# B3zaleel/draco-sharp

Hardware: NVIDIA B200
Metric: decoded points/sec (higher is better)
Workload: dtype i32->f32

## Files before the change

### draco_sharp_b200/csrc/dcb_api.cu

```cuda
#include <cuda_runtime.h>
#include <stdint.h>
#include <stdio.h>
#include <chrono>
#include <thread>
#include <mutex>
#include <memory>
#include <string>
#include <stdlib.h>
#include <string.h>

#include <algorithm>
#include <atomic>
#include <map>
#include <new>
#include <tuple>
#include <vector>

#include "dcb_internal.h"
#include "dcb_kernels.h"
#include "dcb_mesh_host.h"
#include "dcb_walk.h"

namespace {

constexpr uint64_t kFrontPad = 256;
constexpr uint64_t kBackPad = 64;
constexpr uint32_t kNumSMsDefault = 148;
constexpr uint32_t kSmemPerSM = 227 * 1024;
constexpr uint32_t kSmemPerCtaReserve = 1024;
constexpr uint64_t kTabArenaBudget = 1ull << 30;
constexpr uint64_t kDefaultPointsPerByte = 4096;

inline uint64_t align_up(uint64_t v, uint64_t a) { return (v + a - 1) / a * a; }

struct EnvFlags {
  bool no_par_post, no_fanout, debug_plan, debug_timing, lutb_full, rans_pc, no_direct, no_fast_tagged, no_threads;
  int ctas_per_sm, pairs, par_run, rec_ka;
  bool no_rec, split;
  EnvFlags() {
    no_par_post = getenv("DCB_NO_PAR_POST") != nullptr;
    no_fanout = getenv("DCB_NO_FANOUT") != nullptr;
    debug_plan = getenv("DCB_DEBUG_PLAN") != nullptr;
    debug_timing = getenv("DCB_DEBUG_TIMING") != nullptr;
    lutb_full = getenv("DCB_LUTB_FULL") != nullptr;
    rans_pc = getenv("DCB_RANS_PC") != nullptr;
    no_direct = getenv("DCB_NO_DIRECT") != nullptr;
    no_threads = getenv("DCB_NO_THREADS") != nullptr;
    no_fast_tagged = getenv("DCB_NO_FAST_TAGGED") != nullptr;
    ctas_per_sm = getenv("DCB_CTAS_PER_SM") ? atoi(getenv("DCB_CTAS_PER_SM")) : 0;
    pairs = getenv("DCB_PAIRS") ? atoi(getenv("DCB_PAIRS")) : 0;
    par_run = getenv("DCB_PAR_RUN") ? atoi(getenv("DCB_PAR_RUN")) : 0;
    no_rec = getenv("DCB_REC") == nullptr;
    split = getenv("DCB_SPLIT") != nullptr;
    rec_ka = getenv("DCB_REC_KA") ? atoi(getenv("DCB_REC_KA")) : 0;
  }
};
const EnvFlags &env_flags() {
  static const EnvFlags f;
  return f;
}

struct PoolBlock {
  void *p;
  uint64_t bytes;
  int device;
};
struct DevPool {
  std::mutex mu;
  std::vector<PoolBlock> free_blocks;
// ... 72 lines not shown
  int share = 1;
  bool arena_pending = false;
  bool maps_pending = false;
  std::shared_ptr<DevPool> pool;
  uint64_t cap_in = 0, cap_out = 0, cap_aux = 0, cap_maps = 0, cap_stage = 0, cap_streams = 0, cap_walks = 0, cap_order = 0;
  int device = 0;
  std::vector<int> bufs;
  std::vector<StreamDesc> streams, streams0;
  std::vector<BufWalk> walks, walks0;
  std::vector<uint8_t> tags_launched;
  PointStage pstage{};
  uint64_t in_bytes = 0, out_bytes = 0, dbg_bytes = 0, aux_bytes = 0, maps_bytes = 0;
  uint64_t out_base = 0, dbg_base = 0;
  uint8_t *d_in = nullptr, *d_out = nullptr, *d_dbg = nullptr, *d_aux = nullptr, *d_tab = nullptr, *d_maps = nullptr;
  uint64_t tab_cap = 0, dbg_cap = 0;
  StreamDesc *d_streams = nullptr;
  BufWalk *d_walks = nullptr;
  uint32_t *d_order = nullptr;
  uint64_t order_cap = 0;
  uint8_t *h_stage = nullptr;
  uint8_t *h_maps = nullptr;
  uint64_t cap_hmaps = 0;
  uint8_t *h_desc = nullptr;
  uint64_t cap_hdesc = 0;
  bool desc_pending = false;
  std::vector<uint32_t> order_host;
  uint32_t epoch = 0;
  bool uploaded = false, dirty = true, own_out = false;
  uint8_t *ext_out = nullptr, *ext_dbg = nullptr;
  std::vector<uint64_t> fin_off, fin_bytes;
// ... 378 lines not shown
}

void pinned_free(const std::shared_ptr<DevPool> &pool, void *p, uint64_t cap);
void free_shard_device(Shard &sh) {
  if (sh.h_desc) {
    pinned_free(sh.pool, sh.h_desc, sh.cap_hdesc);
    sh.h_desc = nullptr;
    sh.desc_pending = false;
  }
  if (!sh.d_in && !sh.d_streams && !sh.h_stage && !sh.d_out && !sh.h_maps) return;
  cudaSetDevice(sh.device);
  pool_free(sh.pool, sh.device, sh.d_in, sh.cap_in);
  if (sh.own_out) pool_free(sh.pool, sh.device, sh.d_out, sh.cap_out);
  cudaFree(sh.d_dbg);
  pool_free(sh.pool, sh.device, sh.d_aux, sh.cap_aux);
  cudaFree(sh.d_tab);
  pool_free(sh.pool, sh.device, sh.d_maps, sh.cap_maps);
  pool_free(sh.pool, sh.device, sh.d_streams, sh.cap_streams);
  pool_free(sh.pool, sh.device, sh.d_walks, sh.cap_walks);
  pool_free(sh.pool, sh.device, sh.d_order, sh.cap_order);
  pool_free(sh.pool, sh.device, sh.d_pts, sh.cap_pts);
  sh.d_pts = nullptr;
  pool_free(sh.pool, sh.device, sh.d_faces, sh.cap_faces);
  sh.d_faces = nullptr;
  if (sh.h_fstatus) pinned_free(sh.pool, sh.h_fstatus, sh.cap_hfstatus);
  sh.h_fstatus = nullptr;
  if (sh.h_stage) pinned_free(sh.pool, sh.h_stage, sh.cap_stage);
  if (sh.h_maps) pinned_free(sh.pool, sh.h_maps, sh.cap_hmaps);
  sh.h_maps = nullptr;
  sh.d_in = sh.d_out = sh.d_dbg = sh.d_aux = sh.d_tab = sh.d_maps = nullptr;
// ... 498 lines not shown
      const uint32_t blk = std::max(16u, ((1u << g.prec_bits) >> 7) << 2);
      const uint64_t cta_raw = (sm_bytes + 1024 / share) / ctas_per_sm;
      const uint64_t cta_fixed = (uint64_t)kSmemPerCtaReserve + g.lut_bytes + blk + 256;
      const uint64_t cta_budget = cta_raw > cta_fixed ? cta_raw - cta_fixed : 0;
      const uint64_t used = (uint64_t)g.lanes * (lane_bytes + blk);
      if (cta_budget > used) {
        const uint64_t spare = (cta_budget - used) / g.lanes;
        g.lutb_bytes = (uint32_t)std::min<uint64_t>((1u << g.prec_bits) >> 1, spare / 16 * 16);
      }
      if (g.lutb_bytes) {
        const uint32_t need = lutb_need();
        if (need != 0xFFFFFFFFu && !env_flags().lutb_full) g.lutb_bytes = std::min<uint32_t>(g.lutb_bytes, need);
      }
    }
  }
}

int ensure_order(Shard &sh, uint64_t n) {
  if (n <= sh.order_cap) return DCB_OK;
  pool_free(sh.pool, sh.device, sh.d_order, sh.cap_order);
  sh.d_order = nullptr;
  sh.order_cap = 0;
  uint8_t *p = nullptr;
  CUDA_TRY(pool_alloc(sh.pool, sh.device, std::max<uint64_t>(n, 1024) * 4, &p, &sh.cap_order));
  sh.d_order = reinterpret_cast<uint32_t *>(p);
  sh.order_cap = std::max<uint64_t>(n, 1024);
  return DCB_OK;
}

void tl_mark(dcb_ctx *ctx, const std::string &name, cudaStream_t s, bool begin);
// ... 687 lines not shown
    if (key.compact) g.exc = std::max(g.exc, s.n_active - std::min(s.n_active, s.dense_prefix));
    g.total_symbols += s.n_entries;
    g.max_entries = std::max(g.max_entries, s.n_entries);
    g.note_table(s);
    g.order.push_back(si);
  }
  std::vector<Group *> rgs;
  for (auto &kv : raw) rgs.push_back(&kv.second);
  bool side_followers = false;
  for (Group *g : rgs) side_followers = side_followers || (g->mode == 3 && rgs.size() > 1);
  for (Group *g : rgs) {
    g->no_direct = g->force_single_warp;
    for (Group *o : rgs)
      if (o != g && o->order.size() >= (size_t)num_sms * 8) g->no_direct = true;
    std::vector<Group *> one{g};
    plan_rans_groups(one, num_sms, (uint32_t)sh.share, side_followers ? 6u * 1024u : 0u);
  }
  uint64_t n_order = 0;
  auto add = [&](Group &g) {
    g.order_off = n_order;
    n_order += g.order.size();
  };
  for (Group *g : rgs) {
    std::stable_sort(g->order.begin(), g->order.end(),
                     [&](uint32_t x, uint32_t y) { return sh.streams[x].n_entries > sh.streams[y].n_entries; });
    add(*g);
  }
  for (int n = 1; n <= 4; ++n) { add(post[n]); add(para[n]); add(cmp[n]); add(par[n]); }
  add(copy);
  add(octs);
  add(octc);
// ... 81 lines not shown
    for (int n = 1; n <= 4; ++n) all.insert(all.end(), par_runs[n].begin(), par_runs[n].end());

    CUDA_TRY(cudaMemcpyAsync(sh.d_order, all.data(), all.size() * 4, cudaMemcpyHostToDevice, st));
  }
  Group *dom = nullptr;
  for (Group *g : rgs)
    if (!dom || g->total_symbols > dom->total_symbols) dom = g;
  const bool fan_out = rgs.size() > 1 && !env_flags().no_fanout;
  bool flag_kernels = !geo.order.empty();
  for (int n = 1; n <= 4; ++n) flag_kernels = flag_kernels || !cmp[n].order.empty();
  const bool flags_early = flag_kernels && !deferred_descs && !env_flags().no_fanout;
  if (fan_out || flags_early) {
    CUDA_TRY(cudaEventRecord(ctx->fork_ev[dev_index], st));
    for (cudaStream_t ss : ctx->side[dev_index]) CUDA_TRY(cudaStreamWaitEvent(ss, ctx->fork_ev[dev_index], 0));
  }
  bool side_used[3] = {false, false, false};
  size_t gi = 0;
  const cudaStream_t st_main = st;
  for (Group *g : rgs) {
    const uint32_t n = (uint32_t)g->order.size();
    const bool is_dom = timed && dev_index == 0 && g == dom;
    cudaStream_t st = st_main;
    if (fan_out && !g->table_global && (g != dom || g->mode == 3)) {
      const size_t k = g->mode == 3 ? 0 : 1 + gi++ % 2;
      st = ctx->side[dev_index][k];
      side_used[k] = true;
    }
    if (env_flags().debug_plan)
      fprintf(stderr, "[dcb plan] raw group ncp=%d wide=%d compact=%u prec=%u entries=%u mode=%u zig=%u: %u streams, %llu symbols, "
                      "k=%u lut=%uB lutb=%uB ent=%uB lanes=%u pairs=%u split=%u direct=%u global=%d rec_ka=%u rec=%uB (need x8: %u %u %u %u, exc %u)\n",
              g->ncp, (int)g->wide, g->compact, g->prec_bits, g->entries, g->mode, g->zig, n,
              (unsigned long long)g->total_symbols, g->lut_shift, g->lut_bytes, g->lutb_bytes, g->ent_bytes, g->lanes, g->pairs, g->split,
              g->direct, (int)g->table_global, g->rec_ka, g->rec_bytes, g->rec_max[0], g->rec_max[1], g->rec_max[2], g->rec_max[3], g->exc_all);
    if (is_dom) CUDA_TRY(cudaEventRecord(ctx->ev[2], st));
    if (g->table_global) {
      const uint64_t slot_bytes = (uint64_t)g->lut_bytes + g->ent_bytes;
      uint64_t per = std::max<uint64_t>(32, std::min<uint64_t>(kTabArenaBudget / slot_bytes, 0xF0000000ull / slot_bytes) / 32 * 32);
      const uint64_t chunk = std::min<uint64_t>(per, align_up(n, 32));
      if (sh.tab_cap < chunk * slot_bytes) {
        cudaFree(sh.d_tab);
        sh.d_tab = nullptr;
        sh.tab_cap = 0;
        CUDA_TRY(cudaMalloc(&sh.d_tab, chunk * slot_bytes));
        sh.tab_cap = chunk * slot_bytes;
      }
      A.tab = sh.d_tab;
      for (uint64_t o = 0; o < n; o += chunk) {
        RansLaunch L{sh.d_streams, sh.d_order + g->order_off + o, (uint32_t)std::min<uint64_t>(chunk, n - o), 32,
                     g->lut_bytes, 0, g->ent_bytes, g->entries, g->exc, g->lut_shift, g->prec_bits, dump, g->compact, g->zig, 0};
        CUDA_TRY(dcb_launch_rans_raw(L, g->ncp, g->wide, true, A, st));
        stats.n_launches++;
      }
    } else {
      RansLaunch L{sh.d_streams, sh.d_order + g->order_off, n, g->lanes, g->lut_bytes, g->lutb_bytes, g->ent_bytes,
                   g->entries, g->exc, g->lut_shift, g->prec_bits, dump, g->compact, g->zig, g->mode};
      tl_begin(g->mode == 1 ? "rans mode1" : g->mode == 2 ? "rans mode2" : g->mode == 3 ? "rans mode3" : g->mode == 4 ? "rans mode4" : "rans mode0", st);
      L.pairs = g->pairs;
      L.direct = g->direct;
      L.rec_ka = g->rec_ka;
      L.rec_bytes = g->rec_bytes;
      L.split = g->split;
      if (g->rec_ka) L.cap_exc = g->exc_all;
      CUDA_TRY(g->rec_ka ? dcb_launch_rans_raw_rec(L, g->ncp, A, st)
               : g->pairs ? dcb_launch_rans_raw_pc(L, g->ncp, A, st) : dcb_launch_rans_raw(L, g->ncp, g->wide, false, A, st));
      tl_end(st);
      stats.n_launches++;
    }
    if (g->mode == 3) {
      tl_begin("oct_chain", st);
      CUDA_TRY(dcb_launch_oct_chain(sh.d_streams, sh.d_order + g->order_off, n, dump, A, st));
      tl_end(st);
      tl_begin("oct_unit", st);
      CUDA_TRY(dcb_launch_oct_unit(sh.d_streams, sh.d_order + g->order_off, n, g->max_entries, A, st));
      tl_end(st);
      stats.n_launches += 2;
    }
    if (is_dom) {
      CUDA_TRY(cudaEventRecord(ctx->ev[3], st));
      ctx->ev_raw = true;
      for (uint32_t si : g->order) {
        const StreamDesc &sd = sh.streams[si];
// ... 6 lines not shown
      Ls.rec_bytes = g->rec_bytes;
      const uint32_t cta_smem = (g->rec_ka ? dcb_rans_rec_smem_bytes(Ls, 4u * (uint32_t)g->ncp)
                                 : g->pairs ? dcb_rans_pc_smem_bytes(Ls, 4u * (uint32_t)g->ncp) : dcb_rans_smem_bytes(Ls, g->table_global)) + kSmemPerCtaReserve;
      const uint64_t per_wave = (uint64_t)num_sms * std::max<uint32_t>(1u, std::min<uint32_t>(32u, (kSmemPerSM + 1024u) / cta_smem)) * g->lanes * std::max(1u, g->pairs);
      stats.n_waves = g->table_global ? 1 : (int32_t)((n + per_wave - 1) / per_wave);
      if (g->rec_ka)
        snprintf(ctx->raw_name, sizeof ctx->raw_name, "rans_raw_rec<ncp=%d,u16,smem,mode=%u,bucket records 2^%u|16|1,%ux%u lanes,%uB>", g->ncp,
                 g->mode, g->rec_ka, g->pairs, g->lanes, g->rec_bytes);
      else if (g->pairs)
        snprintf(ctx->raw_name, sizeof ctx->raw_name, "rans_raw_pc<ncp=%d,u16,smem,mode=%u,%s,%s,%ux%u lanes>", g->ncp, g->mode,
                 g->direct ? "direct slot LUT" : "two-level LUT", g->compact ? "compact" : "dense", g->pairs, g->lanes);
      else
        snprintf(ctx->raw_name, sizeof ctx->raw_name, "rans_raw_fused<ncp=%d,%s,%s,mode=%u,k=%u,%s>", g->ncp,
                 g->wide ? "u32" : "u16", g->table_global ? "global" : "smem", g->mode, g->lut_shift,
                 g->compact ? "compact" : "dense");
    }
    stats.n_streams += (int32_t)n;
  }
  auto launch_flag_kernels = [&](cudaStream_t fs, cudaStream_t gs) -> int {
    for (int n = 1; n <= 4; ++n)
      if (!cmp[n].order.empty()) {
        CUDA_TRY(dcb_launch_cmp_flags(sh.d_streams, sh.d_order + cmp[n].order_off, (uint32_t)cmp[n].order.size(), A, fs));
        stats.n_launches++;
      }
    if (!geo.order.empty()) {
      CUDA_TRY(dcb_launch_geo_flips(sh.d_streams, sh.d_order + geo.order_off, (uint32_t)geo.order.size(), A, gs));
      stats.n_launches++;
    }
    return DCB_OK;
  };
// ... 7 lines not shown
    if (rcm) return rcm;
  }
  auto launch_cmp_deps = [&](cudaStream_t ds) -> int {
    for (int n = 1; n <= 4; ++n)
      if (!cmp[n].order.empty()) {
        CUDA_TRY(dcb_launch_cmp_deps(sh.d_streams, sh.d_order + cmp[n].order_off, (uint32_t)cmp[n].order.size(), cmp[n].max_entries, A, ds));
        stats.n_launches++;
      }
    return DCB_OK;
  };
  if (flags_early) {
    CUDA_TRY(cudaStreamWaitEvent(ctx->side[dev_index][2], ctx->maps_ev[dev_index], 0));
    int rcd = launch_cmp_deps(ctx->side[dev_index][2]);
    if (rcd) return rcd;
  }
  for (int k = 0; k < 3; ++k)
    if (side_used[k]) {
      CUDA_TRY(cudaEventRecord(ctx->join_ev[dev_index][k], ctx->side[dev_index][k]));
      CUDA_TRY(cudaStreamWaitEvent(st, ctx->join_ev[dev_index][k], 0));
    }
  if (!wide.order.empty()) {
    CUDA_TRY(dcb_launch_wide_post(sh.d_streams, sh.d_order + wide.order_off, (uint32_t)wide.order.size(), dump, A, st));
    stats.n_launches++;
  }
  for (int n = 1; n <= 4; ++n) {
    if (!post[n].order.empty()) {
      CUDA_TRY(dcb_launch_serial_post(sh.d_streams, sh.d_order + post[n].order_off, (uint32_t)post[n].order.size(), n, dump, 0, A, st));
      stats.n_launches++;
    }
    if (!par[n].order.empty()) {
      const uint32_t np = (uint32_t)par[n].order.size();
// ... 384 lines not shown
    for (int dev : c->devices) {
      cudaDeviceProp p;
      if (dev < 0 || dev >= count || cudaGetDeviceProperties(&p, dev) != cudaSuccess || p.major != 10) {
        cudaGetLastError();
        dcb_destroy(c);
        return DCB_ERR_NO_DEVICE;
      }
      cudaStream_t st = nullptr;
      if (cudaSetDevice(dev) != cudaSuccess || cudaStreamCreateWithFlags(&st, cudaStreamNonBlocking) != cudaSuccess) {
        cudaGetLastError();
        dcb_destroy(c);
        return DCB_ERR_CUDA;
      }
      c->streams.push_back(st);
      c->own_stream.push_back(true);
      std::vector<cudaStream_t> side(3, nullptr);
      std::vector<cudaEvent_t> jev(3, nullptr);
      cudaEvent_t fev = nullptr;
      int prio_lo = 0, prio_hi = 0;
      cudaDeviceGetStreamPriorityRange(&prio_lo, &prio_hi);
      for (int k = 0; k < 3; ++k) {
        if (k == 0) cudaStreamCreateWithPriority(&side[k], cudaStreamNonBlocking, prio_hi);
        else cudaStreamCreateWithFlags(&side[k], cudaStreamNonBlocking);
        cudaEventCreateWithFlags(&jev[k], cudaEventDisableTiming);
      }
      cudaEventCreateWithFlags(&fev, cudaEventDisableTiming);
      c->side.push_back(side);
      c->join_ev.push_back(jev);
      c->fork_ev.push_back(fev);
      {
        cudaStream_t ci = nullptr, co = nullptr;
        bool own = true;
        for (size_t e = 0; e + 1 < c->streams.size(); ++e)
          if (c->devices[e] == dev) { ci = c->copy_in[e]; co = c->copy_out[e]; own = false; break; }
        if (own) {
          cudaStreamCreateWithFlags(&ci, cudaStreamNonBlocking);
// ... 493 lines not shown
```

### draco_sharp_b200/csrc/dcb_internal.h

```cpp
#pragma once
#include <stdint.h>

#include "../../include/dracob200.h"

#if defined(__CUDACC__)
#define DCB_HD __host__ __device__ __forceinline__
#else
#define DCB_HD inline
#endif

#define DCB_VARINT_CHUNK 4096u

enum : int32_t {
  DT_INT8 = 1, DT_UINT8 = 2, DT_INT16 = 3, DT_UINT16 = 4, DT_INT32 = 5, DT_UINT32 = 6,
  DT_INT64 = 7, DT_UINT64 = 8, DT_FLOAT32 = 9, DT_FLOAT64 = 10, DT_BOOL = 11, DT_COUNT = 12
};
enum : int32_t { SEQ_GENERIC = 0, SEQ_INTEGER = 1, SEQ_QUANTIZATION = 2, SEQ_NORMALS = 3 };
enum : int32_t {
  PRED_NONE = -2, PRED_DIFFERENCE = 0, PRED_PARALLELOGRAM = 1, PRED_CONSTRAINED_MULTI = 4, PRED_TEX_COORDS_PORTABLE = 5,
  PRED_GEOMETRIC_NORMAL = 6, PRED_COUNT = 7
};
enum : int32_t { XF_NONE = -1, XF_DELTA = 0, XF_WRAP = 1, XF_OCT = 2, XF_OCT_CANON = 3, XF_COUNT = 4 };
enum : uint8_t {
  SCHEME_TAGGED = 0,
// ... 164 lines not shown
  uint32_t lutb_bytes;
  uint32_t ent_bytes;
  uint32_t cap_entries;
  uint32_t cap_exc;
  uint32_t lut_shift;
  uint32_t prec_bits;
  uint32_t dump;
  uint32_t compact;
  uint32_t zig;
  uint32_t mode;
  uint32_t pairs;
  uint32_t direct;
  uint32_t rec_ka;
  uint32_t rec_bytes;
  uint32_t split;
};
```

### draco_sharp_b200/csrc/dcb_kernels.cu

```cuda
#include <cuda_runtime.h>
#include <stdint.h>
#include <algorithm>
#include <stdio.h>
#include <stdlib.h>

#include "dcb_device.cuh"
#include "dcb_internal.h"
#include "dcb_kernels.h"
#include "dcb_walk.h"

using namespace dcb;

namespace {

template <int NCP, typename T, bool DUMP, bool TG, int MODE, int TAB, bool SPLIT>
__device__ __forceinline__ void run_tail(RansLane<T, TG> &rl, const TableGeom &geom, const PostParams &pp, uint8_t *optr,
                                         int32_t *dptr, uint32_t dump, uint32_t n_entries, uint32_t g, int32_t *prev);

template <int NCP, typename T, bool DUMP, bool TG, int MODE, int TAB, bool SPLIT>
__device__ __forceinline__ void run_stream(RansLane<T, TG> &rl, const TableGeom &geom, const PostParams &pp, uint8_t *optr,
                                           int32_t *dptr, uint32_t dump, uint32_t n_entries, uint32_t g_min) {
  const int store = store_of<MODE>(pp), dsize = dsize_of<MODE>(pp);
  int32_t prev[NCP];
#pragma unroll
// ... 74 lines not shown
    while (g + 1 < g_min && rl.bytes_left() >= 2u * kGroupBytes + 4u) {
      lean_sp_group<NCP, MODE, false, 1, true>(rl, pp, optr, g, prev, ca_prev, gate, zero);
      ++g;
      rl.template top_up<(kGroupBytes + 15) / 16 + 1>();
      cp_async_wait<1>();
    }
    lean_sp_group<NCP, MODE, true, 1, true>(rl, pp, optr, g, prev, ca_prev, gate, zero);
    ++g;
    rl.template top_up<(kGroupBytes + 15) / 16 + 1>();
    cp_async_wait<1>();
  }
  rl.prefetch();
  run_tail<NCP, uint16_t, false, false, MODE, 2, true>(rl, geom, pp, optr, nullptr, 0u, n_entries, g, prev);
}

template <int NCP, typename T, bool DUMP, bool TABLE_GLOBAL, int MODE, int TAB>
__global__ void __launch_bounds__(32) rans_raw_fused_kernel(const uint8_t *__restrict__ arena, StreamDesc *streams,
                                                            const uint32_t *__restrict__ order, uint32_t n_streams,
                                                            uint32_t lanes, TableGeom geom, uint8_t *__restrict__ out,
                                                            uint8_t *__restrict__ dbg, uint8_t *__restrict__ aux,
                                                            uint8_t *__restrict__ tab_arena, uint32_t dump) {
  extern __shared__ __align__(16) uint8_t smem[];
  const uint32_t lane = threadIdx.x;
  const uint32_t slot = blockIdx.x * lanes + lane;
  const bool have = lane < lanes && slot < n_streams;
  StreamDesc *dp = have ? &streams[order[slot]] : nullptr;
  const uint32_t smem_base = (uint32_t)__cvta_generic_to_shared(smem);
  const SmemLayout lay = smem_layout(smem_base, lanes, geom, TABLE_GLOBAL);

  RansLane<T, TABLE_GLOBAL> rl;
  uint32_t n_entries = 0;
  T *lut = nullptr, *ent = nullptr;
  uint8_t *lutb = nullptr;
  uint32_t *blk = nullptr;
  bool split_ok = true;
  bool lean_ok = true;
// ... 33 lines not shown
        lean_ok = split_ok && geom.zig != 0 && !(dump & 0x40000000u) &&
                  (MODE == 3 || MODE == 4 ||
                   ((int64_t)rl.max_abs_val < md && d.xf_a >= -(1 << 29) && d.xf_b <= (1 << 29)));
      }
    }
    if (status != DCB_OK) {
      dp->status = status;
      n_entries = 0;
    }
  }
  const bool use_split = __all_sync(0xffffffffu, split_ok);
  const bool use_lean = __all_sync(0xffffffffu, lean_ok);
  uint32_t g_min = n_entries ? (n_entries >> 2) : 0xFFFFFFFFu;
#pragma unroll
  for (int o = 16; o > 0; o >>= 1) g_min = min(g_min, __shfl_xor_sync(0xffffffffu, g_min, o));
  if (n_entries == 0) return;
  rl.fill_lut(geom, lut, lutb, blk, ent, use_split);
  rl.init_ring(smem_base + lay.ring0 + lane * DCB_RING_BYTES);

  PostParams pp;
  pp.load(*dp);
  uint8_t *optr = out + dp->out_off;
  int32_t *dptr = DUMP ? reinterpret_cast<int32_t *>(dbg + dp->dbg_off) : nullptr;
  const bool wide_nc = NCP == 1 && MODE == 0 && dp->ncp > 4;
  if (wide_nc) {
    pp.recon = RECON_NONE;
    dump &= ~(uint32_t)DCB_DUMP_QINTS;
  }
  if (MODE == 3 || MODE == 4 || (MODE == 0 && (pp.recon == RECON_PARA_WRAP || pp.store == STORE_OCT_UNIT || wide_nc))) {
    optr = aux + dp->aux_off;
    if (NCP == 2 && pp.store == STORE_OCT_UNIT) {
      pp.recon = RECON_NONE;
      dump &= ~(uint32_t)DCB_DUMP_QINTS;
    }
    pp.store = STORE_NARROW;
    pp.dsize = 4;
  }
  if constexpr (sizeof(T) == 2 && !TABLE_GLOBAL && !DUMP && MODE >= 1 && MODE <= 4 && TAB == 2) {
    if (use_lean) {
#ifndef DCB_NO_LEAN_SP
      run_stream_lean_sp<NCP, MODE>(rl, geom, pp, optr, n_entries, g_min, blockIdx.y);
      return;
#endif
      if constexpr (MODE == 1 || MODE == 2) {
        run_stream_lean<NCP, MODE>(rl, geom, pp, optr, n_entries, g_min);
        return;
      }
    }
  }
  if (use_split)
    run_stream<NCP, T, DUMP, TABLE_GLOBAL, MODE, TAB, true>(rl, geom, pp, optr, dptr, dump, n_entries, g_min);
  else
    run_stream<NCP, T, DUMP, TABLE_GLOBAL, MODE, TAB, false>(rl, geom, pp, optr, dptr, dump, n_entries, g_min);
}
// ... 564 lines not shown
uint32_t dcb_rans_smem_bytes(const RansLaunch &p, bool table_global) {
  uint32_t b = DCB_RING_BYTES + p.lanes_per_warp * DCB_RING_BYTES;
  if (!table_global && p.direct) return b + 32u + p.lanes_per_warp * (p.lut_bytes + p.ent_bytes);
  if (!table_global) {
    const uint32_t blk = p.lutb_bytes ? std::max(16u, ((1u << p.prec_bits) >> 7) << 2) : 0u;
    b += p.lut_bytes + blk + 16u + p.lanes_per_warp * (p.lut_bytes + p.lutb_bytes + blk + p.ent_bytes);
  }
  return b;
}

static uint32_t no_split_bit() {
  static const uint32_t bit = (getenv("DCB_NO_SPLIT") ? 0x80000000u : 0u) | (getenv("DCB_NO_LEAN") ? 0x40000000u : 0u);
  return bit;
}

template <int NCP, typename T, bool DUMP, bool TG, int MODE, int TAB = 0>
static cudaError_t launch_raw_t(const RansLaunch &p, const DevArenas &a, cudaStream_t st) {
  auto k = rans_raw_fused_kernel<NCP, T, DUMP, TG, MODE, TAB>;
  const uint32_t smem_bytes = dcb_rans_smem_bytes(p, TG);
  if (smem_bytes > 48 * 1024) {
    cudaError_t e = cudaFuncSetAttribute(k, cudaFuncAttributeMaxDynamicSharedMemorySize, (int)smem_bytes);
    if (e != cudaSuccess) return e;
  }
  cudaFuncSetAttribute(k, cudaFuncAttributePreferredSharedMemoryCarveout, (int)cudaSharedmemCarveoutMaxShared);
  const uint32_t grid = (p.n_streams + p.lanes_per_warp - 1) / p.lanes_per_warp;
  k<<<grid, 32, smem_bytes, st>>>(a.in, p.d_streams, p.d_order, p.n_streams, p.lanes_per_warp, geom_of(p), a.out, a.dbg,
                                  a.aux, a.tab, p.dump | no_split_bit());
  return cudaGetLastError();
}

template <int NCP, typename T>
static cudaError_t launch_raw_n(const RansLaunch &p, bool table_global, const DevArenas &a, cudaStream_t st) {
  const bool dump = p.dump != 0;
  if (table_global)
    return dump ? launch_raw_t<NCP, T, true, true, 0>(p, a, st) : launch_raw_t<NCP, T, false, true, 0>(p, a, st);
  return dump ? launch_raw_t<NCP, T, true, false, 0>(p, a, st) : launch_raw_t<NCP, T, false, false, 0>(p, a, st);
}

cudaError_t dcb_launch_rans_raw(const RansLaunch &p, int ncp, bool wide, bool table_global, const DevArenas &a,
                                cudaStream_t st) {
#ifdef DCB_DEV_ONLY_C2
  return launch_raw_t<3, uint16_t, false, false, 1, 2>(p, a, st);
#else
  if (!wide && !table_global && !p.dump) {
#define DCB_SPEC(M, N)                                                                           \
  if (p.mode == M && ncp == N)                                                                   \
    return p.compact ? launch_raw_t<N, uint16_t, false, false, M, 2>(p, a, st)                   \
                     : launch_raw_t<N, uint16_t, false, false, M, 1>(p, a, st);
    DCB_SPEC(1, 3)
    DCB_SPEC(1, 2)
    DCB_SPEC(2, 3)
    DCB_SPEC(2, 4)
    DCB_SPEC(3, 2)
    DCB_SPEC(4, 3)
    DCB_SPEC(4, 2)
#undef DCB_SPEC
  }
#define DCB_CASE(N)                                                       \
// ... 134 lines not shown
```

### draco_sharp_b200/csrc/dcb_kernels.h

```cpp
#pragma once
#include <cuda_runtime.h>
#include <stdint.h>

#include "dcb_internal.h"

#define DCB_TAG_CHUNK 256u
#define DCB_PAR_WARPS 8u
#define DCB_RING_BYTES 128u
#define DCB_PC_STAGES 4u
#define DCB_PC_ROW_BYTES 64u
#define DCB_PC_CTL_BYTES 112u
#define DCB_PC_HAND_BYTES 48u
#define DCB_REC_HAND_BYTES 56u
#define DCB_REC_STAGES 2u
#define DCB_REC_CTL_BYTES 64u
struct PcGeom {
  uint32_t tab_bytes;
  uint32_t slice_bytes;
  uint32_t q_off, ctl_off, hand_off;
  uint32_t fuse;
};

struct DevArenas {
  const uint8_t *in;
  uint8_t *out;
  uint8_t *dbg;
  uint8_t *aux;
  uint8_t *tab;
  const uint8_t *maps;
};

uint32_t dcb_rans_smem_bytes(const RansLaunch &p, bool table_global);
cudaError_t dcb_launch_rans_raw(const RansLaunch &p, int ncp, bool wide, bool table_global, const DevArenas &a,
                                cudaStream_t st);
PcGeom dcb_pc_geom(const RansLaunch &p, uint32_t syms_per_group);
uint32_t dcb_rans_pc_smem_bytes(const RansLaunch &p, uint32_t syms_per_group);
cudaError_t dcb_launch_rans_raw_pc(const RansLaunch &p, int ncp, const DevArenas &a, cudaStream_t st);
cudaError_t dcb_launch_rans_tag_pc(const RansLaunch &p, const DevArenas &a, cudaStream_t st);
uint32_t dcb_rans_rec_smem_bytes(const RansLaunch &p, uint32_t syms_per_group);
cudaError_t dcb_launch_rans_raw_rec(const RansLaunch &p, int ncp, const DevArenas &a, cudaStream_t st);
cudaError_t dcb_launch_rans_tag_rec(const RansLaunch &p, const DevArenas &a, cudaStream_t st);
cudaError_t dcb_launch_rans_tag(const RansLaunch &p, const DevArenas &a, cudaStream_t st);
cudaError_t dcb_launch_resolve(const DevArenas &a, BufWalk *d_walks, const uint32_t *d_list, uint32_t n,
                               StreamDesc *d_streams, cudaStream_t st);
cudaError_t dcb_launch_serial_post(StreamDesc *d_streams, const uint32_t *d_order, uint32_t n, int ncp, uint32_t dump,
                                   uint32_t only_irregular, const DevArenas &a, cudaStream_t st);
uint32_t dcb_par_post_smem_bytes(int ncp);
void dcb_par_post_plan(uint32_t n_streams, uint64_t total_chunks, uint32_t max_chunks, bool any_delta, uint32_t num_sms, int ncp,
                       uint32_t share,
// ... 88 lines not shown
```

Measured before the change: 38.50 billion.

## Split rANS decode into rank producer and concurrent prediction post kernel

```diff
diff --git a/draco_sharp_b200/csrc/dcb_api.cu b/draco_sharp_b200/csrc/dcb_api.cu
--- a/draco_sharp_b200/csrc/dcb_api.cu
+++ b/draco_sharp_b200/csrc/dcb_api.cu
@@ -36,7 +36,7 @@
 struct EnvFlags {
   bool no_par_post, no_fanout, debug_plan, debug_timing, lutb_full, rans_pc, no_direct, no_fast_tagged, no_threads;
   int ctas_per_sm, pairs, par_run, rec_ka;
-  bool no_rec, split;
+  bool no_rec, split, no_chain_split;
   EnvFlags() {
     no_par_post = getenv("DCB_NO_PAR_POST") != nullptr;
     no_fanout = getenv("DCB_NO_FANOUT") != nullptr;
@@ -53,6 +53,7 @@
     no_rec = getenv("DCB_REC") == nullptr;
     split = getenv("DCB_SPLIT") != nullptr;
     rec_ka = getenv("DCB_REC_KA") ? atoi(getenv("DCB_REC_KA")) : 0;
+    no_chain_split = getenv("DCB_NO_CHAIN_SPLIT") != nullptr;
   }
 };
 const EnvFlags &env_flags() {
@@ -155,6 +156,8 @@
   uint64_t out_base = 0, dbg_base = 0;
   uint8_t *d_in = nullptr, *d_out = nullptr, *d_dbg = nullptr, *d_aux = nullptr, *d_tab = nullptr, *d_maps = nullptr;
   uint64_t tab_cap = 0, dbg_cap = 0;
+  uint8_t *d_rank = nullptr;
+  uint64_t cap_rank = 0;
   StreamDesc *d_streams = nullptr;
   BufWalk *d_walks = nullptr;
   uint32_t *d_order = nullptr;
@@ -563,6 +566,9 @@
   if (sh.own_out) pool_free(sh.pool, sh.device, sh.d_out, sh.cap_out);
   cudaFree(sh.d_dbg);
   pool_free(sh.pool, sh.device, sh.d_aux, sh.cap_aux);
+  pool_free(sh.pool, sh.device, sh.d_rank, sh.cap_rank);
+  sh.d_rank = nullptr;
+  sh.cap_rank = 0;
   cudaFree(sh.d_tab);
   pool_free(sh.pool, sh.device, sh.d_maps, sh.cap_maps);
   pool_free(sh.pool, sh.device, sh.d_streams, sh.cap_streams);
@@ -1091,6 +1097,12 @@
       }
     }
   }
+}
+
+constexpr uint64_t kRankScratchBudget = 24ull << 30;
+bool chain_split_shape(const Group &g, int share, uint32_t dump) {
+  return g.kind == 0 && g.mode == 1 && (g.ncp == 2 || g.ncp == 3) && !g.wide && g.compact && share == 1 && !dump &&
+         !env_flags().no_chain_split;
 }
 
 int ensure_order(Shard &sh, uint64_t n) {
@@ -1808,7 +1820,10 @@
     for (Group *o : rgs)
       if (o != g && o->order.size() >= (size_t)num_sms * 8) g->no_direct = true;
     std::vector<Group *> one{g};
-    plan_rans_groups(one, num_sms, (uint32_t)sh.share, side_followers ? 6u * 1024u : 0u);
+    const uint32_t corun = chain_split_shape(*g, sh.share, dump)
+                               ? dcb_rank_post_smem_bytes((uint32_t)g->order.size(), num_sms, g->ncp) + kSmemPerCtaReserve
+                               : 0u;
+    plan_rans_groups(one, num_sms, (uint32_t)sh.share, std::max(corun, side_followers ? 6u * 1024u : 0u));
   }
   uint64_t n_order = 0;
   auto add = [&](Group &g) {
@@ -1920,7 +1935,7 @@
     CUDA_TRY(cudaEventRecord(ctx->fork_ev[dev_index], st));
     for (cudaStream_t ss : ctx->side[dev_index]) CUDA_TRY(cudaStreamWaitEvent(ss, ctx->fork_ev[dev_index], 0));
   }
-  bool side_used[3] = {false, false, false};
+  bool side_used[4] = {false, false, false, false};
   size_t gi = 0;
   const cudaStream_t st_main = st;
   for (Group *g : rgs) {
@@ -1939,6 +1954,7 @@
               (unsigned long long)g->total_symbols, g->lut_shift, g->lut_bytes, g->lutb_bytes, g->ent_bytes, g->lanes, g->pairs, g->split,
               g->direct, (int)g->table_global, g->rec_ka, g->rec_bytes, g->rec_max[0], g->rec_max[1], g->rec_max[2], g->rec_max[3], g->exc_all);
     if (is_dom) CUDA_TRY(cudaEventRecord(ctx->ev[2], st));
+    uint32_t split_rb = 0;
     if (g->table_global) {
       const uint64_t slot_bytes = (uint64_t)g->lut_bytes + g->ent_bytes;
       uint64_t per = std::max<uint64_t>(32, std::min<uint64_t>(kTabArenaBudget / slot_bytes, 0xF0000000ull / slot_bytes) / 32 * 32);
@@ -1967,10 +1983,43 @@
       L.rec_bytes = g->rec_bytes;
       L.split = g->split;
       if (g->rec_ka) L.cap_exc = g->exc_all;
+      if (g == dom && chain_split_shape(*g, sh.share, dump) && !g->pairs && !g->rec_ka && !g->table_global && g->lutb_bytes > 0) {
+        const uint32_t rb = g->entries <= 256 ? 1u : 2u;
+        uint64_t stride = 0;
+        const uint64_t bytes = dcb_rank_scratch_bytes(n, g->max_entries, g->ncp, g->entries, rb, &stride);
+        if (bytes <= kRankScratchBudget) {
+          if (sh.cap_rank < bytes) {
+            pool_free(sh.pool, sh.device, sh.d_rank, sh.cap_rank);
+            sh.d_rank = nullptr;
+            sh.cap_rank = 0;
+            CUDA_TRY(pool_alloc(sh.pool, sh.device, bytes, &sh.d_rank, &sh.cap_rank));
+            CUDA_TRY(cudaMemsetAsync(sh.d_rank, 0, sh.cap_rank, st));
+          }
+          L.rank = sh.d_rank;
+          L.rank_stride = stride;
+          L.rank_vcap = g->entries;
+          L.rank_bytes = rb;
+          L.epoch = next_epoch(sh);
+          split_rb = rb;
+          CUDA_TRY(cudaEventRecord(ctx->fork_ev[dev_index], st));
+          CUDA_TRY(cudaStreamWaitEvent(ctx->side[dev_index][3], ctx->fork_ev[dev_index], 0));
+          if (env_flags().debug_plan)
+            fprintf(stderr, "[dcb plan] chain split: rans_raw_fused ranks=u%u + rank_post_kernel, %u streams, rank scratch %llu B\n",
+                    8u * rb, n, (unsigned long long)bytes);
+        }
+      }
       CUDA_TRY(g->rec_ka ? dcb_launch_rans_raw_rec(L, g->ncp, A, st)
                : g->pairs ? dcb_launch_rans_raw_pc(L, g->ncp, A, st) : dcb_launch_rans_raw(L, g->ncp, g->wide, false, A, st));
       tl_end(st);
       stats.n_launches++;
+      if (split_rb) {
+        cudaStream_t ps = ctx->side[dev_index][3];
+        tl_begin("rank_post", ps);
+        CUDA_TRY(dcb_launch_rank_post(L, g->ncp, num_sms, A, ps));
+        tl_end(ps);
+        side_used[3] = true;
+        stats.n_launches++;
+      }
     }
     if (g->mode == 3) {
       tl_begin("oct_chain", st);
@@ -2007,6 +2056,11 @@
         snprintf(ctx->raw_name, sizeof ctx->raw_name, "rans_raw_fused<ncp=%d,%s,%s,mode=%u,k=%u,%s>", g->ncp,
                  g->wide ? "u32" : "u16", g->table_global ? "global" : "smem", g->mode, g->lut_shift,
                  g->compact ? "compact" : "dense");
+      if (split_rb) {
+        const size_t len = strlen(ctx->raw_name);
+        if (len > 0 && len + 24 < sizeof ctx->raw_name)
+          snprintf(ctx->raw_name + len - 1, sizeof ctx->raw_name - (len - 1), ",ranks u%u>", 8u * split_rb);
+      }
     }
     stats.n_streams += (int32_t)n;
   }
@@ -2044,7 +2098,7 @@
     int rcd = launch_cmp_deps(ctx->side[dev_index][2]);
     if (rcd) return rcd;
   }
-  for (int k = 0; k < 3; ++k)
+  for (int k = 0; k < 4; ++k)
     if (side_used[k]) {
       CUDA_TRY(cudaEventRecord(ctx->join_ev[dev_index][k], ctx->side[dev_index][k]));
       CUDA_TRY(cudaStreamWaitEvent(st, ctx->join_ev[dev_index][k], 0));
@@ -2459,12 +2513,12 @@
       }
       c->streams.push_back(st);
       c->own_stream.push_back(true);
-      std::vector<cudaStream_t> side(3, nullptr);
-      std::vector<cudaEvent_t> jev(3, nullptr);
+      std::vector<cudaStream_t> side(4, nullptr);
+      std::vector<cudaEvent_t> jev(4, nullptr);
       cudaEvent_t fev = nullptr;
       int prio_lo = 0, prio_hi = 0;
       cudaDeviceGetStreamPriorityRange(&prio_lo, &prio_hi);
-      for (int k = 0; k < 3; ++k) {
+      for (int k = 0; k < 4; ++k) {
         if (k == 0) cudaStreamCreateWithPriority(&side[k], cudaStreamNonBlocking, prio_hi);
         else cudaStreamCreateWithFlags(&side[k], cudaStreamNonBlocking);
         cudaEventCreateWithFlags(&jev[k], cudaEventDisableTiming);
diff --git a/draco_sharp_b200/csrc/dcb_internal.h b/draco_sharp_b200/csrc/dcb_internal.h
--- a/draco_sharp_b200/csrc/dcb_internal.h
+++ b/draco_sharp_b200/csrc/dcb_internal.h
@@ -202,4 +202,7 @@
   uint32_t rec_ka;
   uint32_t rec_bytes;
   uint32_t split;
-};
+  uint8_t *rank;
+  uint64_t rank_stride;
+  uint32_t rank_vcap, rank_bytes, epoch;
+};
diff --git a/draco_sharp_b200/csrc/dcb_kernels.cu b/draco_sharp_b200/csrc/dcb_kernels.cu
--- a/draco_sharp_b200/csrc/dcb_kernels.cu
+++ b/draco_sharp_b200/csrc/dcb_kernels.cu
@@ -112,12 +112,78 @@
   run_tail<NCP, uint16_t, false, false, MODE, 2, true>(rl, geom, pp, optr, nullptr, 0u, n_entries, g, prev);
 }
 
-template <int NCP, typename T, bool DUMP, bool TABLE_GLOBAL, int MODE, int TAB>
+#define DCB_RANK_CHUNK 256u
+constexpr uint32_t kRankSkip = 0xFFFFFFFFu;
+
+struct RankArgs {
+  uint64_t *ready;
+  int32_t *vmap;
+  uint8_t *ranks;
+  uint64_t stride;
+  uint32_t vcap;
+  uint32_t epoch;
+};
+
+__device__ __forceinline__ void rank_publish(uint64_t *w, uint32_t epoch, uint32_t v) {
+  asm volatile("st.release.gpu.global.u64 [%0], %1;\n" ::"l"(w), "l"(((uint64_t)epoch << 32) | v) : "memory");
+}
+__device__ __forceinline__ uint64_t rank_poll(const uint64_t *w) {
+  uint64_t v;
+  asm volatile("ld.acquire.gpu.global.u64 %0, [%1];\n" : "=l"(v) : "l"(w) : "memory");
+  return v;
+}
+
+template <int NCP, int RB>
+__device__ __forceinline__ void run_stream_ranks(RansLane<uint16_t, false> &rl, uint8_t *rptr, uint64_t *ready, uint32_t epoch,
+                                                 uint32_t n_entries, uint32_t g_min) {
+  constexpr uint32_t kGroupBytes = 4u * NCP * 3u;
+  constexpr int kSyms = 4 * NCP;
+  constexpr int kWords = 4 * kSyms * RB / 4;
+  static_assert(kWords % 4 == 0, "whole 16-byte stores");
+  uint32_t g = 0;
+  for (; g + 4u <= g_min; g += 4u) {
+    if (rl.bytes_left() < 4u * kGroupBytes) break;
+    uint32_t w[kWords];
+#pragma unroll
+    for (int k = 0; k < kWords; ++k) w[k] = 0u;
+#pragma unroll
+    for (int q = 0; q < 4; ++q) {
+#pragma unroll
+      for (int s = 0; s < kSyms; ++s) {
+        if (s % 3 == 0) rl.window_open();
+        const uint32_t ca = (s % 3 == 0) ? rl.template step_lean<true>() : rl.template step_lean<false>();
+        if (s % 3 == 2 || s == kSyms - 1) rl.window_close();
+        const int i = q * kSyms + s;
+        w[i * RB / 4] |= ((ca - rl.cum_addr) >> 1) << (8 * ((i * RB) % 4));
+      }
+      rl.template top_up<(kGroupBytes + 15) / 16 + 1>();
+      cp_async_wait<1>();
+    }
+    uint4 *o = reinterpret_cast<uint4 *>(rptr + (uint64_t)g * (uint32_t)(kSyms * RB));
+#pragma unroll
+    for (int k = 0; k < kWords / 4; ++k) o[k] = make_uint4(w[4 * k], w[4 * k + 1], w[4 * k + 2], w[4 * k + 3]);
+    if (((g + 4u) & (DCB_RANK_CHUNK / 4u - 1u)) == 0u) rank_publish(ready, epoch, (g + 4u) / (DCB_RANK_CHUNK / 4u));
+  }
+  rl.prefetch();
+  for (uint64_t i = (uint64_t)g * kSyms; i < (uint64_t)n_entries * NCP; i += NCP) {
+#pragma unroll
+    for (int c = 0; c < NCP; ++c) {
+      const uint32_t rank = (rl.template step<true, 1>() - rl.ent_off) >> 1;
+      if (RB == 1) rptr[i + c] = (uint8_t)rank;
+      else reinterpret_cast<uint16_t *>(rptr)[i + c] = (uint16_t)rank;
+    }
+    rl.template top_up<(3 * NCP + 15) / 16 + 1>();
+    cp_async_wait<0>();
+  }
+  rank_publish(ready, epoch, (n_entries + DCB_RANK_CHUNK - 1u) / DCB_RANK_CHUNK);
+}
+
+template <int NCP, typename T, bool DUMP, bool TABLE_GLOBAL, int MODE, int TAB, int RB = 0>
 __global__ void __launch_bounds__(32) rans_raw_fused_kernel(const uint8_t *__restrict__ arena, StreamDesc *streams,
                                                             const uint32_t *__restrict__ order, uint32_t n_streams,
                                                             uint32_t lanes, TableGeom geom, uint8_t *__restrict__ out,
                                                             uint8_t *__restrict__ dbg, uint8_t *__restrict__ aux,
-                                                            uint8_t *__restrict__ tab_arena, uint32_t dump) {
+                                                            uint8_t *__restrict__ tab_arena, uint32_t dump, RankArgs rk) {
   extern __shared__ __align__(16) uint8_t smem[];
   const uint32_t lane = threadIdx.x;
   const uint32_t slot = blockIdx.x * lanes + lane;
@@ -181,6 +247,7 @@
   uint32_t g_min = n_entries ? (n_entries >> 2) : 0xFFFFFFFFu;
 #pragma unroll
   for (int o = 16; o > 0; o >>= 1) g_min = min(g_min, __shfl_xor_sync(0xffffffffu, g_min, o));
+  if (RB > 0 && have && (n_entries == 0 || !use_lean)) rank_publish(rk.ready + slot, rk.epoch, kRankSkip);
   if (n_entries == 0) return;
   rl.fill_lut(geom, lut, lutb, blk, ent, use_split);
   rl.init_ring(smem_base + lay.ring0 + lane * DCB_RING_BYTES);
@@ -205,6 +272,12 @@
   }
   if constexpr (sizeof(T) == 2 && !TABLE_GLOBAL && !DUMP && MODE >= 1 && MODE <= 4 && TAB == 2) {
     if (use_lean) {
+      if constexpr (RB > 0) {
+        int32_t *vm = rk.vmap + (uint64_t)slot * rk.vcap;
+        for (uint32_t r = 0; r < rl.n_entries_tab; ++r) vm[r] = rl.value(rl.ent_off + 2u * r, true, true);
+        run_stream_ranks<NCP, RB>(rl, rk.ranks + (uint64_t)slot * rk.stride, rk.ready + slot, rk.epoch, n_entries, g_min);
+        return;
+      }
 #ifndef DCB_NO_LEAN_SP
       run_stream_lean_sp<NCP, MODE>(rl, geom, pp, optr, n_entries, g_min, blockIdx.y);
       return;
@@ -799,9 +872,182 @@
   return bit;
 }
 
-template <int NCP, typename T, bool DUMP, bool TG, int MODE, int TAB = 0>
+static RankArgs rank_args(const RansLaunch &p) {
+  RankArgs r{};
+  if (!p.rank) return r;
+  const uint64_t ready_bytes = (((uint64_t)p.n_streams * 8u) + 127u) & ~127ull;
+  const uint64_t vmap_bytes = (((uint64_t)p.n_streams * p.rank_vcap * 4u) + 127u) & ~127ull;
+  r.ready = reinterpret_cast<uint64_t *>(p.rank);
+  r.vmap = reinterpret_cast<int32_t *>(p.rank + ready_bytes);
+  r.ranks = p.rank + ready_bytes + vmap_bytes;
+  r.stride = p.rank_stride;
+  r.vcap = p.rank_vcap;
+  r.epoch = p.epoch;
+  return r;
+}
+
+uint64_t dcb_rank_scratch_bytes(uint32_t n_streams, uint32_t max_entries, int ncp, uint32_t vcap, uint32_t rank_bytes,
+                                uint64_t *stride) {
+  const uint64_t chunks = ((uint64_t)max_entries + DCB_RANK_CHUNK - 1u) / DCB_RANK_CHUNK;
+  *stride = ((chunks * DCB_RANK_CHUNK * (uint64_t)ncp * rank_bytes) + 127u) & ~127ull;
+  return ((((uint64_t)n_streams * 8u) + 127u) & ~127ull) + ((((uint64_t)n_streams * vcap * 4u) + 127u) & ~127ull) +
+         (uint64_t)n_streams * *stride;
+}
+
+#define DCB_RANK_POST_WARPS 4u
+
+template <int NCP, int RB>
+__device__ __forceinline__ void rank_post_chunk(const StreamDesc &d, const RankArgs &rk, uint32_t slot, uint32_t k,
+                                                uint32_t *carry, uint8_t *out, uint32_t lane) {
+  __syncwarp();
+  PostParams pp;
+  pp.load(d);
+  const uint32_t md = (uint32_t)pp.max_diff;
+  const uint32_t e0 = k * DCB_RANK_CHUNK + lane * 8u;
+  const uint32_t nv = d.n_entries > e0 ? min(8u, d.n_entries - e0) : 0u;
+  constexpr int kSyms = 8 * NCP;
+  uint32_t w[kSyms * RB / 4];
+  const uint2 *rp = reinterpret_cast<const uint2 *>(rk.ranks + (uint64_t)slot * rk.stride + (uint64_t)e0 * NCP * RB);
+#pragma unroll
+  for (int j = 0; j < kSyms * RB / 8; ++j) {
+    const uint2 v = __ldcg(rp + j);
+    w[2 * j] = v.x;
+    w[2 * j + 1] = v.y;
+  }
+  const int32_t *vm = rk.vmap + (uint64_t)slot * rk.vcap;
+  uint32_t cm[kSyms], res[NCP];
+#pragma unroll
+  for (int c = 0; c < NCP; ++c) res[c] = 0u;
+#pragma unroll
+  for (int i = 0; i < kSyms; ++i) {
+    const uint32_t rank = RB == 1 ? (w[i / 4] >> (8 * (i % 4))) & 0xFFu : (w[i / 2] >> (16 * (i % 2))) & 0xFFFFu;
+    const int32_t corr = (uint32_t)(i / NCP) < nv ? __ldcg(vm + rank) : 0;
+    cm[i] = corr < 0 ? (uint32_t)corr + md : (uint32_t)corr;
+    uint32_t t = res[i % NCP] + cm[i];
+    res[i % NCP] = t >= md ? t - md : t;
+  }
+#pragma unroll
+  for (int c = 0; c < NCP; ++c) {
+    uint32_t x = res[c];
+#pragma unroll
+    for (int o = 1; o < 32; o <<= 1) {
+      const uint32_t y = __shfl_up_sync(0xffffffffu, x, o);
+      if (lane >= (uint32_t)o) {
+        x += y;
+        if (x >= md) x -= md;
+      }
+    }
+    const uint32_t total = __shfl_sync(0xffffffffu, x, 31);
+    uint32_t acc = x >= res[c] ? x - res[c] : x + md - res[c];
+    acc += carry[c];
+    if (acc >= md) acc -= md;
+    res[c] = acc;
+    const uint32_t nc = carry[c] + total;
+    __syncwarp();
+    if (lane == 0) carry[c] = nc >= md ? nc - md : nc;
+  }
+  float f[kSyms];
+#pragma unroll
+  for (int i = 0; i < kSyms; ++i) {
+    const int c = i % NCP;
+    uint32_t t = res[c] + cm[i];
+    res[c] = t >= md ? t - md : t;
+    f[i] = pp.dequant((int32_t)((uint32_t)pp.mn + res[c]), c);
+  }
+  float *o = reinterpret_cast<float *>(out + d.out_off) + (uint64_t)e0 * NCP;
+  if (nv == 8u) {
+#pragma unroll
+    for (int j = 0; j < kSyms / 4; ++j)
+      reinterpret_cast<float4 *>(o)[j] = make_float4(f[4 * j], f[4 * j + 1], f[4 * j + 2], f[4 * j + 3]);
+  } else {
+#pragma unroll
+    for (int i = 0; i < kSyms; ++i)
+      if ((uint32_t)(i / NCP) < nv) o[i] = f[i];
+  }
+}
+
+template <int NCP, int RB>
+__global__ void __launch_bounds__(DCB_RANK_POST_WARPS * 32) rank_post_kernel(const StreamDesc *__restrict__ streams,
+                                                                            const uint32_t *__restrict__ order, uint32_t n_streams,
+                                                                            uint32_t per_warp, RankArgs rk, uint8_t *__restrict__ out) {
+  extern __shared__ uint32_t rank_smem[];
+  const uint32_t lane = threadIdx.x & 31u, warp = threadIdx.x >> 5;
+  const uint32_t n_warps = gridDim.x * DCB_RANK_POST_WARPS, wg = blockIdx.x * DCB_RANK_POST_WARPS + warp;
+  uint32_t *state = rank_smem + warp * per_warp * (1u + NCP);
+  const uint32_t mine = wg < n_streams ? (n_streams - wg + n_warps - 1u) / n_warps : 0u;
+  for (uint32_t j = lane; j < mine; j += 32u) {
+    const StreamDesc &d = streams[order[wg + j * n_warps]];
+    state[j * (1u + NCP)] = 0u;
+    const int32_t mn = d.xf_a, mx = d.xf_b;
+    const int32_t p0 = 0 > mx ? mx : (0 < mn ? mn : 0);
+#pragma unroll
+    for (int c = 0; c < NCP; ++c) state[j * (1u + NCP) + 1u + c] = (uint32_t)p0 - (uint32_t)mn;
+  }
+  __syncwarp();
+  uint32_t left = mine;
+  while (left > 0) {
+    bool moved = false;
+    for (uint32_t base = 0; base < mine; base += 32u) {
+      const uint32_t j = base + lane;
+      uint32_t avail = 0u, done = kRankSkip;
+      if (j < mine) {
+        done = state[j * (1u + NCP)];
+        if (done != kRankSkip) {
+          const uint64_t v = rank_poll(rk.ready + wg + j * n_warps);
+          if ((uint32_t)(v >> 32) == rk.epoch) avail = (uint32_t)v;
+        }
+      }
+      uint32_t ready = __ballot_sync(0xffffffffu, done != kRankSkip && avail != 0u && avail != done);
+      while (ready) {
+        const uint32_t l = __ffs(ready) - 1u;
+        ready &= ready - 1u;
+        const uint32_t jj = base + l, slot = wg + jj * n_warps;
+        const uint32_t a = __shfl_sync(0xffffffffu, avail, l);
+        uint32_t *stj = state + jj * (1u + NCP);
+        const StreamDesc &d = streams[order[slot]];
+        const uint32_t n_chunks = (d.n_entries + DCB_RANK_CHUNK - 1u) / DCB_RANK_CHUNK;
+        if (a == kRankSkip) {
+          if (lane == 0) stj[0] = kRankSkip;
+        } else {
+          (void)rank_poll(rk.ready + slot);
+          for (uint32_t k = stj[0]; k < a; ++k) rank_post_chunk<NCP, RB>(d, rk, slot, k, stj + 1, out, lane);
+          __syncwarp();
+          if (lane == 0) stj[0] = a == n_chunks ? kRankSkip : a;
+        }
+        __syncwarp();
+        if (stj[0] == kRankSkip) --left;
+        moved = true;
+      }
+    }
+    if (!moved) __nanosleep(2000);
+  }
+}
+
+template <int NCP, int RB>
+static cudaError_t launch_rank_post_t(const RansLaunch &p, uint32_t num_sms, const DevArenas &a, cudaStream_t st) {
+  const uint32_t grid = std::max(1u, std::min(num_sms, (p.n_streams + DCB_RANK_POST_WARPS - 1u) / DCB_RANK_POST_WARPS));
+  const uint32_t per_warp = (p.n_streams + grid * DCB_RANK_POST_WARPS - 1u) / (grid * DCB_RANK_POST_WARPS);
+  const uint32_t smem = DCB_RANK_POST_WARPS * per_warp * (1u + NCP) * 4u;
+  if (smem > 48 * 1024) return cudaErrorInvalidValue;
+  rank_post_kernel<NCP, RB><<<grid, DCB_RANK_POST_WARPS * 32, smem, st>>>(p.d_streams, p.d_order, p.n_streams, per_warp,
+                                                                         rank_args(p), a.out);
+  return cudaGetLastError();
+}
+
+uint32_t dcb_rank_post_smem_bytes(uint32_t n_streams, uint32_t num_sms, int ncp) {
+  const uint32_t warps = std::max(1u, num_sms) * DCB_RANK_POST_WARPS;
+  return DCB_RANK_POST_WARPS * ((n_streams + warps - 1u) / warps) * (1u + (uint32_t)ncp) * 4u;
+}
+
+cudaError_t dcb_launch_rank_post(const RansLaunch &p, int ncp, uint32_t num_sms, const DevArenas &a, cudaStream_t st) {
+  if (ncp == 3) return p.rank_bytes == 1 ? launch_rank_post_t<3, 1>(p, num_sms, a, st) : launch_rank_post_t<3, 2>(p, num_sms, a, st);
+  if (ncp == 2) return p.rank_bytes == 1 ? launch_rank_post_t<2, 1>(p, num_sms, a, st) : launch_rank_post_t<2, 2>(p, num_sms, a, st);
+  return cudaErrorInvalidValue;
+}
+
+template <int NCP, typename T, bool DUMP, bool TG, int MODE, int TAB = 0, int RB = 0>
 static cudaError_t launch_raw_t(const RansLaunch &p, const DevArenas &a, cudaStream_t st) {
-  auto k = rans_raw_fused_kernel<NCP, T, DUMP, TG, MODE, TAB>;
+  auto k = rans_raw_fused_kernel<NCP, T, DUMP, TG, MODE, TAB, RB>;
   const uint32_t smem_bytes = dcb_rans_smem_bytes(p, TG);
   if (smem_bytes > 48 * 1024) {
     cudaError_t e = cudaFuncSetAttribute(k, cudaFuncAttributeMaxDynamicSharedMemorySize, (int)smem_bytes);
@@ -810,7 +1056,7 @@
   cudaFuncSetAttribute(k, cudaFuncAttributePreferredSharedMemoryCarveout, (int)cudaSharedmemCarveoutMaxShared);
   const uint32_t grid = (p.n_streams + p.lanes_per_warp - 1) / p.lanes_per_warp;
   k<<<grid, 32, smem_bytes, st>>>(a.in, p.d_streams, p.d_order, p.n_streams, p.lanes_per_warp, geom_of(p), a.out, a.dbg,
-                                  a.aux, a.tab, p.dump | no_split_bit());
+                                  a.aux, a.tab, p.dump | no_split_bit(), rank_args(p));
   return cudaGetLastError();
 }
 
@@ -827,6 +1073,14 @@
 #ifdef DCB_DEV_ONLY_C2
   return launch_raw_t<3, uint16_t, false, false, 1, 2>(p, a, st);
 #else
+  if (p.rank) {
+    if (wide || table_global || p.dump || p.mode != 1 || !p.compact) return cudaErrorInvalidValue;
+    if (ncp == 3) return p.rank_bytes == 1 ? launch_raw_t<3, uint16_t, false, false, 1, 2, 1>(p, a, st)
+                                           : launch_raw_t<3, uint16_t, false, false, 1, 2, 2>(p, a, st);
+    if (ncp == 2) return p.rank_bytes == 1 ? launch_raw_t<2, uint16_t, false, false, 1, 2, 1>(p, a, st)
+                                           : launch_raw_t<2, uint16_t, false, false, 1, 2, 2>(p, a, st);
+    return cudaErrorInvalidValue;
+  }
   if (!wide && !table_global && !p.dump) {
 #define DCB_SPEC(M, N)                                                                           \
   if (p.mode == M && ncp == N)                                                                   \
diff --git a/draco_sharp_b200/csrc/dcb_kernels.h b/draco_sharp_b200/csrc/dcb_kernels.h
--- a/draco_sharp_b200/csrc/dcb_kernels.h
+++ b/draco_sharp_b200/csrc/dcb_kernels.h
@@ -33,6 +33,10 @@
 uint32_t dcb_rans_smem_bytes(const RansLaunch &p, bool table_global);
 cudaError_t dcb_launch_rans_raw(const RansLaunch &p, int ncp, bool wide, bool table_global, const DevArenas &a,
                                 cudaStream_t st);
+uint64_t dcb_rank_scratch_bytes(uint32_t n_streams, uint32_t max_entries, int ncp, uint32_t vcap, uint32_t rank_bytes,
+                                uint64_t *stride);
+uint32_t dcb_rank_post_smem_bytes(uint32_t n_streams, uint32_t num_sms, int ncp);
+cudaError_t dcb_launch_rank_post(const RansLaunch &p, int ncp, uint32_t num_sms, const DevArenas &a, cudaStream_t st);
 PcGeom dcb_pc_geom(const RansLaunch &p, uint32_t syms_per_group);
 uint32_t dcb_rans_pc_smem_bytes(const RansLaunch &p, uint32_t syms_per_group);
 cudaError_t dcb_launch_rans_raw_pc(const RansLaunch &p, int ncp, const DevArenas &a, cudaStream_t st);
```

After: 29.31 billion, median of 6. 23.9% lower.
